# shaderko/velocity-asr

Measured on AMD Instinct MI355X. Metric: audio-sec/sec (RTFx) + frames/s, 5M model batch=32×10s @ 1/2/4/8 MI355X, higher is better.
Workload: dtype f32

## Files before the change

velocity-asr_amd/csrc/gemm_rows.hip:

```cpp
#include <type_traits>

#include "gemm_common.h"
#include "gemm_split.h"

namespace vasr {
namespace {

using namespace gemm;

typedef __attribute__((address_space(3))) void lds_void;

__device__ __forceinline__ void glds16(const void* src, void* dst_base) {
    const unsigned lds = (unsigned)(uintptr_t)(lds_void*)dst_base;
    unsigned keep;
    asm volatile("s_mov_b32 %0, m0\n\ts_mov_b32 m0, %1\n\ts_nop 0\n\tglobal_load_lds_dwordx4 %2, off\n\ts_mov_b32 m0, %0"
                 : "=&s"(keep) : "s"(lds), "v"(src) : "memory");
}

template <int N>
__device__ __forceinline__ void wait_vmcnt() {
    static_assert(N >= 0 && N < 64, "vmcnt range");
    __builtin_amdgcn_s_waitcnt((N & 15) | ((N >> 4) << 14) | (7 << 4) | (15 << 8));
}

#ifndef VASR_ROWS_ABLATE
#define VASR_ROWS_ABLATE 0
#endif
#ifndef VASR_ROWS_WAVES
#define VASR_ROWS_WAVES 8
#endif
#ifndef VASR_ROWS_DEPTH
#define VASR_ROWS_DEPTH 2
#endif
#ifndef VASR_ROWS_STORE_AUX
#define VASR_ROWS_STORE_AUX 2
#endif
constexpr int RW = VASR_ROWS_WAVES;
constexpr int DEPTH = VASR_ROWS_DEPTH;
constexpr int NSLOT = DEPTH + 1;
#ifndef VASR_ROWS_STORE_WAIT
#define VASR_ROWS_STORE_WAIT 1
#endif
#ifndef VASR_ROWS_MAX_GROUP
#define VASR_ROWS_MAX_GROUP 16
#endif
constexpr int MAX_GROUP = VASR_ROWS_MAX_GROUP;

__device__ __forceinline__ void wait_vmcnt_rt(int n) {
    switch (n) {
#define VASR_W(I) case I: wait_vmcnt<I>(); break;
#define VASR_W8(B) VASR_W(B) VASR_W(B + 1) VASR_W(B + 2) VASR_W(B + 3) VASR_W(B + 4) VASR_W(B + 5) VASR_W(B + 6) VASR_W(B + 7)
        VASR_W8(0) VASR_W8(8) VASR_W8(16) VASR_W8(24) VASR_W8(32) VASR_W8(40) VASR_W8(48) VASR_W8(56)
#undef VASR_W8
#undef VASR_W
        default: wait_vmcnt<0>();
    }
}

#ifdef VASR_ROWS_STAMPS
__device__ unsigned long long* g_rows_stamps;
#define VASR_STAMP(v) const unsigned long long v = __builtin_amdgcn_s_memtime()
#else
#define VASR_STAMP(v)
#endif

constexpr int NST = 16;
constexpr int OOB = 0x7FFFFFFC;

template <int EPI>
__device__ __forceinline__ void rows_epilogue(const GemmParams& p, __amdgpu_buffer_rsrc_t cbuf, int m0, int n0,
                                              const floatx16& acc, int r, int h, const float* __restrict__ bias_s,
                                              const float4* __restrict__ qp_s, int cfirst) {
    const int col = n0 + r;
    const bool col_ok = col < p.N;
    const int lc = col - cfirst;
    const float bv = p.bias ? bias_s[lc] : 0.0f;
    float4 qc = make_float4(0.f, 0.f, 0.f, 0.f);
    if (p.qp) qc = qp_s[lc];
    if constexpr (EPI == VASR_EPI_ARGMAX) {
        const int slot = n0 / 32;
#pragma unroll
        for (int i = 0; i < 16; ++i) {
            const int row = m0 + (i & 3) + 8 * (i >> 2) + 4 * h;
            float v = acc[i];
            if (p.bias) v = v + bv;
            if (p.qp) v = fake_quant(v, qc);
            const unsigned u = __float_as_uint(v);
            const unsigned ord = (u & 0x80000000u) ? ~u : (u | 0x80000000u);
            const unsigned long long k0 = col_ok ? ((unsigned long long)ord << 32) | (0xFFFFFFFFu - (unsigned)col) : 0ull;
            const unsigned long long key = gemm::max_u64_over_32_lanes(k0);
            const int off = (r == 31 && row < p.M) ? (row * (int)p.ldc + slot) * 8 : OOB;
            typedef unsigned u32x2 __attribute__((ext_vector_type(2)));
            const u32x2 kv = {(unsigned)key, (unsigned)(key >> 32)};
            if (!(VASR_ROWS_ABLATE & 2)) __builtin_amdgcn_raw_buffer_store_b64(kv, cbuf, off, 0, VASR_ROWS_STORE_AUX);
        }
        return;
    }
    auto body = [&](auto SPc) {
        constexpr int SP = decltype(SPc)::value;
        const bool sp = SP == 1 || (SP == 2 && col >= p.n_out);
#pragma unroll
        for (int i = 0; i < 16; ++i) {
            const int row = m0 + (i & 3) + 8 * (i >> 2) + 4 * h;
            const bool ok = col_ok && row < p.M;
            float v = acc[i];
            if (p.bias) v = v + bv;
            if (p.qp) v = fake_quant(v, qc);
            if constexpr (EPI == VASR_EPI_GELU) {
                v = gelu_fast(v);
            } else if constexpr (EPI == VASR_EPI_SOFTPLUS_FROM) {
                if constexpr (SP == 1) v = softplus20_fast(v);
                else if constexpr (SP == 2) v = sp ? softplus20_fast(v) : v;
            } else if constexpr (EPI == VASR_EPI_RESIDUAL) {
                v = v + p.aux[(int64_t)min(row, p.M - 1) * p.ld_aux + min(col, p.N - 1)];
            } else if constexpr (EPI == VASR_EPI_GELU_PE) {
                v = gelu_fast(v) + p.aux[(int64_t)min(row, p.M - 1) * p.ld_aux + min(col, p.N - 1)];
            }
            if (!(VASR_ROWS_ABLATE & 2))
                __builtin_amdgcn_raw_buffer_store_b32(__float_as_uint(v), cbuf, ok ? (row * (int)p.ldc + col) * 4 : OOB,
                                                      0, VASR_ROWS_STORE_AUX);
        }
    };
    if constexpr (EPI == VASR_EPI_SOFTPLUS_FROM) {
        if (n0 >= p.n_out) body(std::integral_constant<int, 1>());
        else if (n0 + 32 <= p.n_out) body(std::integral_constant<int, 0>());
        else body(std::integral_constant<int, 2>());
    } else {
        body(std::integral_constant<int, 0>());
    }
}

template <int KS, int EPI>
__global__ __launch_bounds__(64 * RW, 1) void gemm_rows_kernel(GemmParams p, int n_groups, int chunks_per_group) {
    constexpr int CHUNK = KS * 3 * 1024;
    constexpr int DW = 4;
    constexpr int NDMA = 3 * KS / DW;
    static_assert((3 * KS) % DW == 0 && RW % DW == 0, "whole DMA pieces per loader wave");
    __shared__ __attribute__((aligned(16))) char wb0[CHUNK];
    __shared__ __attribute__((aligned(16))) char wb1[CHUNK];
    __shared__ __attribute__((aligned(16))) char wb2[CHUNK];
    __shared__ __attribute__((aligned(16))) char wb3[NSLOT > 3 ? CHUNK : 16];
    __shared__ float bias_s[MAX_GROUP * 32];
    __shared__ float4 qp_s[MAX_GROUP * 32];

    const int nblk = (int)gridDim.x;
    const int id = blockIdx.x;
    const int q8 = nblk / 8, r8 = nblk % 8, xg = id % 8;
    const int w = (xg < r8 ? xg * (q8 + 1) : r8 * (q8 + 1) + (xg - r8) * q8) + id / 8;
    const int rb = w / n_groups, ng = w - rb * n_groups;
    const int NT = (p.N + 31) / 32;
    const int c0 = ng * chunks_per_group;
    const int nc = min(chunks_per_group, NT - c0);
    if (nc <= 0) return;

    const int tid = threadIdx.x;
    const int lane = tid & 63;
    const int wave = tid >> 6;
    const int r = lane & 31, h = lane >> 5;
    const int wave_u = __builtin_amdgcn_readfirstlane(wave);
    const int m0 = rb * 32 * RW + wave * 32;
    const int cfirst = c0 * 32;

    const float* __restrict__ arow = p.A + (int64_t)min(m0 + r, p.M - 1) * p.lda;
    float4 xa[KS][2];
#pragma unroll
    for (int ks = 0; ks < KS; ++ks)
#pragma unroll
        for (int u = 0; u < 2; ++u) {
            const int k = 16 * ks + 8 * h + 4 * u;
            const float4 v = *reinterpret_cast<const float4*>(arow + min(k, p.K - 4));
            xa[ks][u] = k < p.K ? v : make_float4(0.f, 0.f, 0.f, 0.f);
        }
    for (int i = tid; i < nc * 32; i += 64 * RW) {
        const int col = min(cfirst + i, p.N - 1);
        if (p.bias) bias_s[i] = p.bias[col];
        if (p.qp) qp_s[i] = p.qp[col];
    }
    bf16x8 a[KS][3];
#pragma unroll
    for (int ks = 0; ks < KS; ++ks) split8(xa[ks][0], xa[ks][1], a[ks][0], a[ks][1], a[ks][2]);

    const char* __restrict__ Wx = reinterpret_cast<const char*>(p.Wx);
    auto slot = [&](int i) -> char* { return i == 0 ? wb0 : i == 1 ? wb1 : i == 2 ? wb2 : wb3; };
    const bool loader = wave_u < DW;
    auto issue = [&](int j) {
        if (!loader) return;
        const char* src = Wx + (int64_t)(c0 + j) * CHUNK + lane * 16;
        char* dst = slot(j % NSLOT);
#pragma unroll
        for (int i = 0; i < NDMA; ++i) {
            const int piece = i * DW + wave_u;
            glds16(src + piece * 1024, dst + piece * 1024);
        }
    };
    for (int j = 0; j < DEPTH && j < nc; ++j) issue(j);

    const int c_bytes = (EPI == VASR_EPI_ARGMAX ? 8 : 4) * ((p.M - 1) * (int)p.ldc + (EPI == VASR_EPI_ARGMAX ? NT : p.N));
    const __amdgpu_buffer_rsrc_t cbuf = __builtin_amdgcn_make_buffer_rsrc(p.C, 0, c_bytes, 0x00020000);
    floatx16 acc[2];
#ifdef VASR_ROWS_STAMPS
    unsigned long long st_wait = 0, st_bar = 0, st_epi = 0, st_dma = 0, st_mfma = 0;
    VASR_STAMP(st_begin);
#endif
    auto step = [&](auto Sc, int j) {
        constexpr int S = decltype(Sc)::value;
        int n_vm = 0;
        if (!loader && !(VASR_ROWS_ABLATE & 2)) n_vm = VASR_ROWS_STORE_WAIT ? NST * max(0, j - max(j - DEPTH + 1, 1)) : 63;
        VASR_STAMP(t0);
        wait_vmcnt_rt(min(n_vm, 63));
        VASR_STAMP(t1);
        if (!(VASR_ROWS_ABLATE & 8)) __builtin_amdgcn_s_barrier();
        VASR_STAMP(t2);
        const char* wb = slot((VASR_ROWS_ABLATE & 4) ? min(j, DEPTH - 1) : j % NSLOT) + lane * 16;
        bf16x8 wf[2][3];
#pragma unroll
        for (int pl = 0; pl < 3; ++pl) wf[0][pl] = *reinterpret_cast<const bf16x8*>(wb + pl * 1024);
        if (j >= 1) rows_epilogue<EPI>(p, cbuf, m0, (c0 + j - 1) * 32, acc[S ^ 1], r, h, bias_s, qp_s, cfirst);
        VASR_STAMP(t3);
        if (j + DEPTH < nc && !(VASR_ROWS_ABLATE & 4)) issue(j + DEPTH);
        VASR_STAMP(t4);
        floatx16 c;
#pragma unroll
        for (int i = 0; i < 16; ++i) c[i] = 0.f;
#pragma unroll
        for (int ks = 0; ks < KS; ++ks) {
            const int cur = ks & 1;
            if (ks + 1 < KS) {
#pragma unroll
                for (int pl = 0; pl < 3; ++pl)
                    wf[cur ^ 1][pl] = *reinterpret_cast<const bf16x8*>(wb + ((ks + 1) * 3 + pl) * 1024);
            }
            __builtin_amdgcn_sched_barrier(0);
            if constexpr (VASR_ROWS_ABLATE & 1) {
                c[0] += (float)a[ks][0][0] * (float)wf[cur][0][0] + (float)a[ks][2][1] * (float)wf[cur][2][1];
                continue;
            }
            c = __builtin_amdgcn_mfma_f32_32x32x16_bf16(a[ks][2], wf[cur][0], c, 0, 0, 0);
            c = __builtin_amdgcn_mfma_f32_32x32x16_bf16(a[ks][0], wf[cur][2], c, 0, 0, 0);
            c = __builtin_amdgcn_mfma_f32_32x32x16_bf16(a[ks][1], wf[cur][1], c, 0, 0, 0);
            c = __builtin_amdgcn_mfma_f32_32x32x16_bf16(a[ks][1], wf[cur][0], c, 0, 0, 0);
            c = __builtin_amdgcn_mfma_f32_32x32x16_bf16(a[ks][0], wf[cur][1], c, 0, 0, 0);
            c = __builtin_amdgcn_mfma_f32_32x32x16_bf16(a[ks][0], wf[cur][0], c, 0, 0, 0);
            __builtin_amdgcn_sched_barrier(0);
        }
        acc[S] = c;
#ifdef VASR_ROWS_STAMPS
        VASR_STAMP(t5);
        st_wait += t1 - t0;
        st_bar += t2 - t1;
        st_epi += t3 - t2;
        st_dma += t4 - t3;
        st_mfma += t5 - t4;
#endif
    };
    for (int j = 0; j < nc; j += 2) {
        step(std::integral_constant<int, 0>(), j);
        if (j + 1 < nc) step(std::integral_constant<int, 1>(), j + 1);
    }
    const int jl = nc - 1;
    rows_epilogue<EPI>(p, cbuf, m0, (c0 + jl) * 32, (jl & 1) ? acc[1] : acc[0], r, h, bias_s, qp_s, cfirst);
#ifdef VASR_ROWS_STAMPS
    __builtin_amdgcn_s_waitcnt(0);
    VASR_STAMP(st_end);
    if (lane == 0 && g_rows_stamps) {
        unsigned long long* o = g_rows_stamps + ((int64_t)blockIdx.x * RW + wave) * 8;
        o[0] = st_wait; o[1] = st_bar; o[2] = st_epi; o[3] = st_dma; o[4] = st_mfma; o[5] = st_end - st_begin;
        o[6] = (unsigned long long)nc; o[7] = loader ? 1 : 0;
    }
#endif
}

#ifndef VASR_ROWS_ROLES
#define VASR_ROWS_ROLES 1
#endif
#ifndef VASR_ROWS_INTERLEAVE
#define VASR_ROWS_INTERLEAVE 1
#endif
#ifndef VASR_ROWS_EPI_FIRST
#define VASR_ROWS_EPI_FIRST 1
#endif
#ifndef VASR_ROWS_DMA_WAVES
#define VASR_ROWS_DMA_WAVES 4
#endif
constexpr int CWV = 4;
constexpr int MWV = 4;
constexpr int DWV = VASR_ROWS_DMA_WAVES;
constexpr int SWV = DWV == MWV ? MWV : MWV - DWV;
static_assert(DWV == 4 || DWV == 2, "VASR_ROWS_DMA_WAVES: 4 or 2");
constexpr int OOB16 = 0x7FFFFFF0;

__device__ __forceinline__ void role_barrier() {
    asm volatile("" ::: "memory");
    __builtin_amdgcn_s_barrier();
    asm volatile("" ::: "memory");
}

template <int CTRL>
__device__ __forceinline__ float dpp_f32(float v) {
    const int i = (int)__float_as_uint(v);
    return __uint_as_float((unsigned)__builtin_amdgcn_update_dpp(i, i, CTRL, 0xF, 0xF, false));
}

template <int EPI, int SP>
__device__ __forceinline__ float rows_value(const GemmParams& p, float v, float bv, const float4& qc, int row, int col) {
    if (p.bias) v = v + bv;
    if (p.qp) v = fake_quant(v, qc);
    if constexpr (EPI == VASR_EPI_GELU) {
        v = gelu_fast(v);
    } else if constexpr (EPI == VASR_EPI_SOFTPLUS_FROM) {
        if constexpr (SP == 1) v = softplus20_fast(v);
        else if constexpr (SP == 2) v = col >= p.n_out ? softplus20_fast(v) : v;
    } else if constexpr (EPI == VASR_EPI_RESIDUAL) {
        v = v + p.aux[(int64_t)min(row, p.M - 1) * p.ld_aux + min(col, p.N - 1)];
    } else if constexpr (EPI == VASR_EPI_GELU_PE) {
        v = gelu_fast(v) + p.aux[(int64_t)min(row, p.M - 1) * p.ld_aux + min(col, p.N - 1)];
    }
    return v;
}

template <int EPI>
__device__ __forceinline__ void roles_epilogue(const GemmParams& p, __amdgpu_buffer_rsrc_t cbuf, int m0, int n0,
                                               const float* __restrict__ tile, int lane, bool wide,
                                               const float* __restrict__ bias_s, const float4* __restrict__ qp_s,
                                               int cfirst) {
    const int rl = lane >> 3, c4 = 4 * (lane & 7);
    const int col0 = n0 + c4;
    const int lc = col0 - cfirst;
    float bv[4] = {0.f, 0.f, 0.f, 0.f};
    if (p.bias) {
        const float4 b = *reinterpret_cast<const float4*>(bias_s + lc);
        bv[0] = b.x; bv[1] = b.y; bv[2] = b.z; bv[3] = b.w;
    }
    float4 qc[4];
#pragma unroll
    for (int e = 0; e < 4; ++e) qc[e] = p.qp ? qp_s[lc + e] : make_float4(0.f, 0.f, 0.f, 0.f);
    if constexpr (EPI == VASR_EPI_ARGMAX) {
        const int slot = n0 / 32;
#pragma unroll
        for (int s = 0; s < 4; ++s) {
            const int row = m0 + 8 * s + rl;
            const float4 x = *reinterpret_cast<const float4*>(tile + (8 * s + rl) * 32 + c4);
            const float xv[4] = {x.x, x.y, x.z, x.w};
            unsigned long long key = 0ull;
#pragma unroll
            for (int e = 0; e < 4; ++e) {
                float v = xv[e];
                if (p.bias) v = v + bv[e];
                if (p.qp) v = fake_quant(v, qc[e]);
                const unsigned u = __float_as_uint(v);
                const unsigned ord = (u & 0x80000000u) ? ~u : (u | 0x80000000u);
                const unsigned long long k =
                    col0 + e < p.N ? ((unsigned long long)ord << 32) | (0xFFFFFFFFu - (unsigned)(col0 + e)) : 0ull;
                key = k > key ? k : key;
            }
            unsigned long long o = gemm::dpp_u64<0xB1, 0xF>(key);
            key = o > key ? o : key;
            o = gemm::dpp_u64<0x4E, 0xF>(key);
            key = o > key ? o : key;
            o = gemm::dpp_u64<0x141, 0xF>(key);
            key = o > key ? o : key;
            const int off = (c4 == 0 && row < p.M) ? (row * (int)p.ldc + slot) * 8 : OOB16;
            typedef unsigned u32x2 __attribute__((ext_vector_type(2)));
            const u32x2 kv = {(unsigned)key, (unsigned)(key >> 32)};
            __builtin_amdgcn_raw_buffer_store_b64(kv, cbuf, off, 0, VASR_ROWS_STORE_AUX);
        }
        return;
    }
    if constexpr (EPI == VASR_EPI_LSE) {
        const int slot = n0 / 32;
#pragma unroll
        for (int s = 0; s < 4; ++s) {
            const int row = m0 + 8 * s + rl;
            const float4 x = *reinterpret_cast<const float4*>(tile + (8 * s + rl) * 32 + c4);
            const float xv[4] = {x.x, x.y, x.z, x.w};
            float v[4];
            float m = -INFINITY;
#pragma unroll
            for (int e = 0; e < 4; ++e) {
                v[e] = col0 + e < p.N ? xv[e] + bv[e] : -INFINITY;
                m = fmaxf(m, v[e]);
            }
            m = fmaxf(m, dpp_f32<0xB1>(m));
            m = fmaxf(m, dpp_f32<0x4E>(m));
            m = fmaxf(m, dpp_f32<0x141>(m));
            const float ms = m == -INFINITY ? 0.f : m;
            float sum = 0.f;
#pragma unroll
            for (int e = 0; e < 4; ++e) sum += fast_exp(v[e] - ms);
            sum += dpp_f32<0xB1>(sum);
            sum += dpp_f32<0x4E>(sum);
            sum += dpp_f32<0x141>(sum);
            const int off = (c4 == 0 && row < p.M) ? (row * (int)p.ldc + slot) * 8 : OOB16;
            typedef unsigned u32x2 __attribute__((ext_vector_type(2)));
            const u32x2 kv = {__float_as_uint(m), __float_as_uint(sum)};
            __builtin_amdgcn_raw_buffer_store_b64(kv, cbuf, off, 0, VASR_ROWS_STORE_AUX);
        }
        return;
    }
    if constexpr (EPI == VASR_EPI_ARGMAX_LSE) {
        const int slot = 2 * (n0 / 32);
#pragma unroll
        for (int s = 0; s < 4; ++s) {
            const int row = m0 + 8 * s + rl;
            const float4 x = *reinterpret_cast<const float4*>(tile + (8 * s + rl) * 32 + c4);
            const float xv[4] = {x.x, x.y, x.z, x.w};
            unsigned long long key = 0ull;
            float v[4];
            float m = -INFINITY;
#pragma unroll
            for (int e = 0; e < 4; ++e) {
                float kvl = xv[e];
                if (p.bias) kvl = kvl + bv[e];
                const unsigned u = __float_as_uint(kvl);
                const unsigned ord = (u & 0x80000000u) ? ~u : (u | 0x80000000u);
                const unsigned long long k =
                    col0 + e < p.N ? ((unsigned long long)ord << 32) | (0xFFFFFFFFu - (unsigned)(col0 + e)) : 0ull;
                key = k > key ? k : key;
                v[e] = col0 + e < p.N ? xv[e] + bv[e] : -INFINITY;
                m = fmaxf(m, v[e]);
            }
            unsigned long long o = gemm::dpp_u64<0xB1, 0xF>(key);
            key = o > key ? o : key;
            o = gemm::dpp_u64<0x4E, 0xF>(key);
            key = o > key ? o : key;
            o = gemm::dpp_u64<0x141, 0xF>(key);
            key = o > key ? o : key;
            m = fmaxf(m, dpp_f32<0xB1>(m));
            m = fmaxf(m, dpp_f32<0x4E>(m));
            m = fmaxf(m, dpp_f32<0x141>(m));
            const float ms = m == -INFINITY ? 0.f : m;
            float sum = 0.f;
#pragma unroll
            for (int e = 0; e < 4; ++e) sum += fast_exp(v[e] - ms);
            sum += dpp_f32<0xB1>(sum);
            sum += dpp_f32<0x4E>(sum);
            sum += dpp_f32<0x141>(sum);
            const bool on = c4 == 0 && row < p.M;
            const int off = on ? (row * (int)p.ldc + slot) * 8 : OOB16;
            typedef unsigned u32x2 __attribute__((ext_vector_type(2)));
            const u32x2 kv = {(unsigned)key, (unsigned)(key >> 32)};
            const u32x2 pv = {__float_as_uint(m), __float_as_uint(sum)};
            __builtin_amdgcn_raw_buffer_store_b64(kv, cbuf, off, 0, VASR_ROWS_STORE_AUX);
            __builtin_amdgcn_raw_buffer_store_b64(pv, cbuf, on ? off + 8 : OOB16, 0, VASR_ROWS_STORE_AUX);
        }
        return;
    }
    auto body = [&](auto SPc, auto Wc) {
        constexpr int SP = decltype(SPc)::value;
        constexpr bool WIDE = decltype(Wc)::value;
#pragma unroll
        for (int s = 0; s < 4; ++s) {
            const int row = m0 + 8 * s + rl;
            const float4 x = *reinterpret_cast<const float4*>(tile + (8 * s + rl) * 32 + c4);
            float v[4] = {x.x, x.y, x.z, x.w};
#pragma unroll
            for (int e = 0; e < 4; ++e) v[e] = rows_value<EPI, SP>(p, v[e], bv[e], qc[e], row, col0 + e);
            if constexpr (WIDE) {
                typedef unsigned u32x4 __attribute__((ext_vector_type(4)));
                const u32x4 d = {__float_as_uint(v[0]), __float_as_uint(v[1]), __float_as_uint(v[2]), __float_as_uint(v[3])};
                const int off = (row < p.M && col0 < p.N) ? (row * (int)p.ldc + col0) * 4 : OOB16;
                if (!(VASR_ROWS_ABLATE & 2) || s == 3) __builtin_amdgcn_raw_buffer_store_b128(d, cbuf, off, 0, VASR_ROWS_STORE_AUX);
            } else {
#pragma unroll
                for (int e = 0; e < 4; ++e)
                    __builtin_amdgcn_raw_buffer_store_b32(__float_as_uint(v[e]), cbuf,
                                                          (row < p.M && col0 + e < p.N) ? (row * (int)p.ldc + col0 + e) * 4 : OOB,
                                                          0, VASR_ROWS_STORE_AUX);
            }
        }
    };
    auto width = [&](auto SPc) {
        if (wide) body(SPc, std::true_type());
        else body(SPc, std::false_type());
    };
    if constexpr (EPI == VASR_EPI_SOFTPLUS_FROM) {
        if (n0 >= p.n_out) width(std::integral_constant<int, 1>());
        else if (n0 + 32 <= p.n_out) width(std::integral_constant<int, 0>());
        else width(std::integral_constant<int, 2>());
    } else {
        width(std::integral_constant<int, 0>());
    }
}

template <int KS, int EPI>
__global__ __launch_bounds__(64 * (CWV + MWV), 1) void gemm_rows_roles_kernel(GemmParams p, int n_groups,
                                                                              int chunks_per_group, int wide) {
    constexpr int CHUNK = KS * 3 * 1024;
    constexpr int NDMA = 3 * KS / DWV;
    static_assert((3 * KS) % DWV == 0, "whole DMA pieces per DMA wave");
    static_assert(DEPTH == 2, "the roles kernel's ring is three slots, two chunks ahead");
    __shared__ __attribute__((aligned(16))) char wb0[CHUNK];
    __shared__ __attribute__((aligned(16))) char wb1[CHUNK];
    __shared__ __attribute__((aligned(16))) char wb2[CHUNK];
    __shared__ __attribute__((aligned(16))) float stage[CWV][2][1024];
    __shared__ __attribute__((aligned(16))) float bias_s[MAX_GROUP * 32];
    __shared__ float4 qp_s[MAX_GROUP * 32];

    const int nblk = (int)gridDim.x;
    const int id = blockIdx.x;
    const int q8 = nblk / 8, r8 = nblk % 8, xg = id % 8;
    const int w = (xg < r8 ? xg * (q8 + 1) : r8 * (q8 + 1) + (xg - r8) * q8) + id / 8;
    const int rb = w / n_groups, ng = w - rb * n_groups;
    const int NT = (p.N + 31) / 32;
    constexpr bool IL = VASR_ROWS_INTERLEAVE != 0;
    const int c0 = IL ? ng : ng * chunks_per_group, cstep = IL ? n_groups : 1;
    const int nc = IL ? (NT - ng + n_groups - 1) / n_groups : min(chunks_per_group, NT - c0);
    if (nc <= 0) return;

    const int tid = threadIdx.x;
    const int lane = tid & 63;
    const int wave_u = __builtin_amdgcn_readfirstlane(tid >> 6);
    auto slot = [&](int i) -> char* { return i == 0 ? wb0 : i == 1 ? wb1 : wb2; };
#ifdef VASR_ROWS_STAMPS
    unsigned long long st_wait = 0, st_bar = 0, st_epi = 0, st_dma = 0, st_mfma = 0;
    VASR_STAMP(st_begin);
#endif

    if (wave_u < CWV) {
        const int r = lane & 31, h = lane >> 5;
        const int m0 = rb * 32 * CWV + wave_u * 32;
        const float* __restrict__ arow = p.A + (int64_t)min(m0 + r, p.M - 1) * p.lda;
        float4 xa[KS][2];
#pragma unroll
        for (int ks = 0; ks < KS; ++ks)
#pragma unroll
            for (int u = 0; u < 2; ++u) {
                const int k = 16 * ks + 8 * h + 4 * u;
                const float4 v = *reinterpret_cast<const float4*>(arow + min(k, p.K - 4));
                xa[ks][u] = k < p.K ? v : make_float4(0.f, 0.f, 0.f, 0.f);
            }
        bf16x8 a[KS][3];
#pragma unroll
        for (int ks = 0; ks < KS; ++ks) split8(xa[ks][0], xa[ks][1], a[ks][0], a[ks][1], a[ks][2]);
        for (int j = 0; j < nc; ++j) {
            VASR_STAMP(t0);
            role_barrier();
            VASR_STAMP(t1);
            const char* wb = slot(j % NSLOT) + lane * 16;
            bf16x8 wf[2][3];
#pragma unroll
            for (int pl = 0; pl < 3; ++pl) wf[0][pl] = *reinterpret_cast<const bf16x8*>(wb + pl * 1024);
            floatx16 c;
#pragma unroll
            for (int i = 0; i < 16; ++i) c[i] = 0.f;
#pragma unroll
            for (int ks = 0; ks < KS; ++ks) {
                const int cur = ks & 1;
                if (ks + 1 < KS) {
#pragma unroll
                    for (int pl = 0; pl < 3; ++pl)
                        wf[cur ^ 1][pl] = *reinterpret_cast<const bf16x8*>(wb + ((ks + 1) * 3 + pl) * 1024);
                }
                __builtin_amdgcn_sched_barrier(0);
                c = __builtin_amdgcn_mfma_f32_32x32x16_bf16(a[ks][2], wf[cur][0], c, 0, 0, 0);
                c = __builtin_amdgcn_mfma_f32_32x32x16_bf16(a[ks][0], wf[cur][2], c, 0, 0, 0);
                c = __builtin_amdgcn_mfma_f32_32x32x16_bf16(a[ks][1], wf[cur][1], c, 0, 0, 0);
                c = __builtin_amdgcn_mfma_f32_32x32x16_bf16(a[ks][1], wf[cur][0], c, 0, 0, 0);
                c = __builtin_amdgcn_mfma_f32_32x32x16_bf16(a[ks][0], wf[cur][1], c, 0, 0, 0);
                c = __builtin_amdgcn_mfma_f32_32x32x16_bf16(a[ks][0], wf[cur][0], c, 0, 0, 0);
                __builtin_amdgcn_sched_barrier(0);
            }
            VASR_STAMP(t2);
            float* tile = &stage[wave_u][j & 1][0];
#pragma unroll
            for (int i = 0; i < 16; ++i) tile[((i & 3) + 8 * (i >> 2) + 4 * h) * 32 + r] = c[i];
            __builtin_amdgcn_s_waitcnt(0xC07F);
#ifdef VASR_ROWS_STAMPS
            VASR_STAMP(t3);
            st_bar += t1 - t0;
            st_mfma += t2 - t1;
            st_epi += t3 - t2;
#endif
        }
        VASR_STAMP(t4);
        role_barrier();
#ifdef VASR_ROWS_STAMPS
        VASR_STAMP(t5);
        st_bar += t5 - t4;
#endif
    } else {
        const int mw = wave_u - CWV;
        const bool dma = mw < DWV;
        const bool stores = mw >= MWV - SWV;
        const int sw = mw - (MWV - SWV);
        for (int i = tid - 64 * CWV; i < nc * 32; i += 64 * MWV) {
            const int col = min((c0 + (i >> 5) * cstep) * 32 + (i & 31), p.N - 1);
            if (p.bias) bias_s[i] = p.bias[col];
            if (p.qp) qp_s[i] = p.qp[col];
        }
        const char* __restrict__ Wx = reinterpret_cast<const char*>(p.Wx);
        auto issue = [&](int j) {
            const char* src = Wx + (int64_t)(c0 + j * cstep) * CHUNK + lane * 16;
            char* dst = slot(j % NSLOT);
#pragma unroll
            for (int i = 0; i < NDMA; ++i) {
                const int piece = i * DWV + mw;
                glds16(src + piece * 1024, dst + piece * 1024);
            }
        };
        __builtin_amdgcn_s_waitcnt(0xC07F);
        if (dma)
            for (int j = 0; j < DEPTH && j < nc; ++j) issue(j);
        constexpr bool SLOTS = EPI == VASR_EPI_ARGMAX || EPI == VASR_EPI_LSE || EPI == VASR_EPI_ARGMAX_LSE;
        constexpr int PER = EPI == VASR_EPI_ARGMAX_LSE ? 2 : 1;
        const int c_bytes = (SLOTS ? 8 : 4) * ((p.M - 1) * (int)p.ldc + (SLOTS ? PER * NT : p.N));
        const __amdgpu_buffer_rsrc_t cbuf = __builtin_amdgcn_make_buffer_rsrc(p.C, 0, c_bytes, 0x00020000);
        auto epilogue = [&](int j) {
            if (!stores) return;
            const int n0 = (c0 + j * cstep) * 32;
            for (int cw = sw; cw < CWV; cw += SWV)
                roles_epilogue<EPI>(p, cbuf, rb * 32 * CWV + cw * 32, n0, &stage[cw][j & 1][0], lane, wide != 0,
                                    bias_s, qp_s, n0 - j * 32);
        };
        for (int j = 0; j < nc; ++j) {
            VASR_STAMP(t0);
            if (dma) {
                if (j + 1 < nc) wait_vmcnt<NDMA*(DEPTH - 1)>();
                else wait_vmcnt<0>();
            }
            VASR_STAMP(t1);
            role_barrier();
            VASR_STAMP(t2);
            if (VASR_ROWS_EPI_FIRST && j >= 1) epilogue(j - 1);
            VASR_STAMP(t2e);
            if (dma && j + DEPTH < nc && !(VASR_ROWS_ABLATE & 4)) issue(j + DEPTH);
            VASR_STAMP(t3);
            if (!VASR_ROWS_EPI_FIRST && j >= 1) epilogue(j - 1);
#ifdef VASR_ROWS_STAMPS
            VASR_STAMP(t4);
            st_wait += t1 - t0;
            st_bar += t2 - t1;
            st_dma += t3 - t2e;
            st_epi += (t2e - t2) + (t4 - t3);
#endif
        }
        VASR_STAMP(t5);
        role_barrier();
        VASR_STAMP(t6);
        epilogue(nc - 1);
#ifdef VASR_ROWS_STAMPS
        VASR_STAMP(t7);
        st_bar += t6 - t5;
        st_epi += t7 - t6;
#endif
    }
#ifdef VASR_ROWS_STAMPS
    __builtin_amdgcn_s_waitcnt(0);
    VASR_STAMP(st_end);
    if (lane == 0 && g_rows_stamps) {
        unsigned long long* o = g_rows_stamps + ((int64_t)blockIdx.x * (CWV + MWV) + wave_u) * 8;
        o[0] = st_wait; o[1] = st_bar; o[2] = st_epi; o[3] = st_dma; o[4] = st_mfma; o[5] = st_end - st_begin;
        o[6] = (unsigned long long)nc;
        o[7] = wave_u < CWV ? 2 : DWV == MWV ? 3 : wave_u - CWV < DWV ? 4 : 5;
    }
#endif
}

inline void pick_groups(int row_blocks, int NT, int* groups_out, int* per_out) {
    int groups = 1, per = min(NT, MAX_GROUP), best = -1;
    for (int g = 1; g <= NT; ++g) {
        const int pg = (NT + g - 1) / g;
        if (pg > MAX_GROUP) continue;
        const int gg = (NT + pg - 1) / pg;
        const int cost = ((row_blocks * gg + kCUs - 1) / kCUs) * (pg + 1);
        if (best < 0 || cost < best) {
            best = cost;
            groups = gg;
            per = pg;
        }
    }
    *groups_out = groups;
    *per_out = per;
}

template <int KS>
int launch_roles(const GemmParams& p, int epi, hipStream_t s) {
    const int NT = (p.N + 31) / 32;
    const int row_blocks = (p.M + 32 * CWV - 1) / (32 * CWV);
    int groups, per;
    pick_groups(row_blocks, NT, &groups, &per);
    const int wide = epi != VASR_EPI_ARGMAX && epi != VASR_EPI_LSE && epi != VASR_EPI_ARGMAX_LSE && p.N % 4 == 0 && p.ldc % 4 == 0 && (reinterpret_cast<uintptr_t>(p.C) & 15) == 0;
    const dim3 grid(row_blocks * groups), block(64 * (CWV + MWV));
#define VASR_R(E) hipLaunchKernelGGL((gemm_rows_roles_kernel<KS, E>), grid, block, 0, s, p, groups, per, wide)
    switch (epi) {
        case VASR_EPI_NONE: VASR_R(VASR_EPI_NONE); break;
        case VASR_EPI_GELU: VASR_R(VASR_EPI_GELU); break;
        case VASR_EPI_SOFTPLUS_FROM: VASR_R(VASR_EPI_SOFTPLUS_FROM); break;
        case VASR_EPI_RESIDUAL: VASR_R(VASR_EPI_RESIDUAL); break;
        case VASR_EPI_GELU_PE: VASR_R(VASR_EPI_GELU_PE); break;
        case VASR_EPI_ARGMAX: VASR_R(VASR_EPI_ARGMAX); break;
        case VASR_EPI_LSE: VASR_R(VASR_EPI_LSE); break;
        case VASR_EPI_ARGMAX_LSE: VASR_R(VASR_EPI_ARGMAX_LSE); break;
        default: set_error("vasr_linear_x3_f32: rows engine: epilogue %d not supported", epi); return VASR_EINVAL;
    }
#undef VASR_R
    return launch_status("vasr_linear_x3_f32");
}

template <int KS>
int launch_rows(const GemmParams& p, int epi, hipStream_t s) {
    const int NT = (p.N + 31) / 32;
    const int row_blocks = (p.M + 32 * RW - 1) / (32 * RW);
    int groups, per;
    pick_groups(row_blocks, NT, &groups, &per);
    const dim3 grid(row_blocks * groups), block(64 * RW);
#define VASR_R(E) hipLaunchKernelGGL((gemm_rows_kernel<KS, E>), grid, block, 0, s, p, groups, per)
    switch (epi) {
        case VASR_EPI_NONE: VASR_R(VASR_EPI_NONE); break;
        case VASR_EPI_GELU: VASR_R(VASR_EPI_GELU); break;
        case VASR_EPI_SOFTPLUS_FROM: VASR_R(VASR_EPI_SOFTPLUS_FROM); break;
        case VASR_EPI_RESIDUAL: VASR_R(VASR_EPI_RESIDUAL); break;
        case VASR_EPI_GELU_PE: VASR_R(VASR_EPI_GELU_PE); break;
        case VASR_EPI_ARGMAX: VASR_R(VASR_EPI_ARGMAX); break;
        default: set_error("vasr_linear_x3_f32: rows engine: epilogue %d not supported", epi); return VASR_EINVAL;
    }
#undef VASR_R
    return launch_status("vasr_linear_x3_f32");
}

}

bool rows_x3_selected(int M, int N, int Kp, int64_t ldc, int batch, int epi) {
    if (batch != 1 || Kp > 192 || M <= 0 || epi == VASR_EPI_PAIR_POWER || epi == VASR_EPI_PAIR_FUSION) return false;
    if ((epi == VASR_EPI_LSE || epi == VASR_EPI_ARGMAX_LSE) && !VASR_ROWS_ROLES) return false;
    if (Kp != 128 && Kp != 192) return false;
    const bool slots = epi == VASR_EPI_ARGMAX || epi == VASR_EPI_LSE || epi == VASR_EPI_ARGMAX_LSE;
    if ((int64_t)M * ldc * (slots ? 8 : 4) >= ((int64_t)1 << 31) - 64) return false;
    const int engine = option(VASR_OPT_GEMM_ENGINE);
    if (engine == 1) return false;
    if (engine == 0 && (Kp != 192 || N < 512 || M < 4096 ||
                        !(epi == VASR_EPI_NONE || epi == VASR_EPI_GELU || epi == VASR_EPI_SOFTPLUS_FROM ||
                          epi == VASR_EPI_LSE)))
        return false;
    return true;
}

int launch_rows_x3(const GemmParams& p, int epi, hipStream_t s) {
    const bool roles = VASR_ROWS_ROLES != 0;
    if (roles) return p.Kp == 128 ? launch_roles<8>(p, epi, s) : launch_roles<12>(p, epi, s);
    return p.Kp == 128 ? launch_rows<8>(p, epi, s) : launch_rows<12>(p, epi, s);
}

}

#ifdef VASR_ROWS_STAMPS
VASR_API int vasr_diag_rows_stamps(void* buf) {
    return hipMemcpyToSymbol(HIP_SYMBOL(vasr::g_rows_stamps), &buf, sizeof(buf)) == hipSuccess ? VASR_OK : VASR_EINVAL;
}
#endif
```

Before: 179,600.

## Stage A tile through LDS, double-buffer accumulators, move softplus epilogue math into compute waves

The A-operand prologue now loads coalesced 64-column passes into a swizzled LDS image and then reads per-lane fragments, instead of strided per-row global loads. A double-accumulator path lets compute waves write the previous chunk's tile interleaved with the current chunk's MFMAs, and the store waves lag by two chunks. For the softplus epilogue without fake-quant, bias and softplus are applied by the compute waves, so the store waves only write raw values. This spreads epilogue arithmetic across MFMA latency but adds register pressure and scheduling constraints.

New measurement: 181,800 (median of 6 runs). 1.01x the previous value.

```diff
diff --git a/velocity-asr_amd/csrc/gemm_rows.hip b/velocity-asr_amd/csrc/gemm_rows.hip
--- a/velocity-asr_amd/csrc/gemm_rows.hip
+++ b/velocity-asr_amd/csrc/gemm_rows.hip
@@ -270,6 +270,18 @@
 #endif
 }
 
+#ifndef VASR_ROWS_A_STAGE
+#define VASR_ROWS_A_STAGE 1
+#endif
+#ifndef VASR_ROWS_ACC2
+#define VASR_ROWS_ACC2 0
+#endif
+#ifndef VASR_ROWS_EPI_MATH
+#define VASR_ROWS_EPI_MATH 1
+#endif
+#ifndef VASR_ROWS_HEAD_ARGMAX
+#define VASR_ROWS_HEAD_ARGMAX 0
+#endif
 #ifndef VASR_ROWS_ROLES
 #define VASR_ROWS_ROLES 1
 #endif
@@ -318,7 +330,7 @@
     return v;
 }
 
-template <int EPI>
+template <int EPI, bool RAW = false>
 __device__ __forceinline__ void roles_epilogue(const GemmParams& p, __amdgpu_buffer_rsrc_t cbuf, int m0, int n0,
                                                const float* __restrict__ tile, int lane, bool wide,
                                                const float* __restrict__ bias_s, const float4* __restrict__ qp_s,
@@ -327,13 +339,13 @@
     const int col0 = n0 + c4;
     const int lc = col0 - cfirst;
     float bv[4] = {0.f, 0.f, 0.f, 0.f};
-    if (p.bias) {
+    if (!RAW && p.bias) {
         const float4 b = *reinterpret_cast<const float4*>(bias_s + lc);
         bv[0] = b.x; bv[1] = b.y; bv[2] = b.z; bv[3] = b.w;
     }
     float4 qc[4];
 #pragma unroll
-    for (int e = 0; e < 4; ++e) qc[e] = p.qp ? qp_s[lc + e] : make_float4(0.f, 0.f, 0.f, 0.f);
+    for (int e = 0; e < 4; ++e) qc[e] = !RAW && p.qp ? qp_s[lc + e] : make_float4(0.f, 0.f, 0.f, 0.f);
     if constexpr (EPI == VASR_EPI_ARGMAX) {
         const int slot = n0 / 32;
 #pragma unroll
@@ -453,8 +465,10 @@
             const int row = m0 + 8 * s + rl;
             const float4 x = *reinterpret_cast<const float4*>(tile + (8 * s + rl) * 32 + c4);
             float v[4] = {x.x, x.y, x.z, x.w};
-#pragma unroll
-            for (int e = 0; e < 4; ++e) v[e] = rows_value<EPI, SP>(p, v[e], bv[e], qc[e], row, col0 + e);
+            if constexpr (!RAW) {
+#pragma unroll
+                for (int e = 0; e < 4; ++e) v[e] = rows_value<EPI, SP>(p, v[e], bv[e], qc[e], row, col0 + e);
+            }
             if constexpr (WIDE) {
                 typedef unsigned u32x4 __attribute__((ext_vector_type(4)));
                 const u32x4 d = {__float_as_uint(v[0]), __float_as_uint(v[1]), __float_as_uint(v[2]), __float_as_uint(v[3])};
@@ -473,7 +487,7 @@
         if (wide) body(SPc, std::true_type());
         else body(SPc, std::false_type());
     };
-    if constexpr (EPI == VASR_EPI_SOFTPLUS_FROM) {
+    if constexpr (EPI == VASR_EPI_SOFTPLUS_FROM && !RAW) {
         if (n0 >= p.n_out) width(std::integral_constant<int, 1>());
         else if (n0 + 32 <= p.n_out) width(std::integral_constant<int, 0>());
         else width(std::integral_constant<int, 2>());
@@ -482,13 +496,17 @@
     }
 }
 
-template <int KS, int EPI>
+template <int KS, int EPI, bool CMATH = false>
 __global__ __launch_bounds__(64 * (CWV + MWV), 1) void gemm_rows_roles_kernel(GemmParams p, int n_groups,
                                                                               int chunks_per_group, int wide) {
     constexpr int CHUNK = KS * 3 * 1024;
     constexpr int NDMA = 3 * KS / DWV;
     static_assert((3 * KS) % DWV == 0, "whole DMA pieces per DMA wave");
     static_assert(DEPTH == 2, "the roles kernel's ring is three slots, two chunks ahead");
+    constexpr bool SLOTS = EPI == VASR_EPI_ARGMAX || EPI == VASR_EPI_LSE || EPI == VASR_EPI_ARGMAX_LSE;
+    static_assert(!CMATH || EPI == VASR_EPI_SOFTPLUS_FROM, "compute-wave arithmetic: the softplus epilogue only");
+    constexpr bool ACC2 = VASR_ROWS_ACC2 == 2 || (VASR_ROWS_ACC2 == 1 && SLOTS) || CMATH;
+    constexpr int LAG = ACC2 ? 2 : 1;
     __shared__ __attribute__((aligned(16))) char wb0[CHUNK];
     __shared__ __attribute__((aligned(16))) char wb1[CHUNK];
     __shared__ __attribute__((aligned(16))) char wb2[CHUNK];
@@ -519,19 +537,181 @@
     if (wave_u < CWV) {
         const int r = lane & 31, h = lane >> 5;
         const int m0 = rb * 32 * CWV + wave_u * 32;
-        const float* __restrict__ arow = p.A + (int64_t)min(m0 + r, p.M - 1) * p.lda;
-        float4 xa[KS][2];
-#pragma unroll
-        for (int ks = 0; ks < KS; ++ks)
-#pragma unroll
-            for (int u = 0; u < 2; ++u) {
-                const int k = 16 * ks + 8 * h + 4 * u;
-                const float4 v = *reinterpret_cast<const float4*>(arow + min(k, p.K - 4));
-                xa[ks][u] = k < p.K ? v : make_float4(0.f, 0.f, 0.f, 0.f);
-            }
         bf16x8 a[KS][3];
-#pragma unroll
-        for (int ks = 0; ks < KS; ++ks) split8(xa[ks][0], xa[ks][1], a[ks][0], a[ks][1], a[ks][2]);
+#if VASR_ROWS_A_STAGE
+        {
+            static_assert(KS % 4 == 0, "whole 64-column passes");
+            constexpr int NP = KS / 4;
+            char* img = reinterpret_cast<char*>(&stage[wave_u][0][0]);
+            const int lq = lane >> 4, lc = lane & 15;
+            float4 g[NP][8];
+#pragma unroll
+            for (int i = 0; i < 8; ++i) {
+                const float* __restrict__ src = p.A + (int64_t)min(m0 + 4 * i + lq, p.M - 1) * p.lda;
+#pragma unroll
+                for (int ps = 0; ps < NP; ++ps) {
+                    const int k = 64 * ps + 4 * lc;
+                    const float4 v = *reinterpret_cast<const float4*>(src + min(k, p.K - 4));
+                    g[ps][i] = k < p.K ? v : make_float4(0.f, 0.f, 0.f, 0.f);
+                }
+            }
+#pragma unroll
+            for (int ps = 0; ps < NP; ++ps) {
+#pragma unroll
+                for (int i = 0; i < 8; ++i) {
+                    const int q = 4 * i + lq;
+                    *reinterpret_cast<float4*>(img + q * 256 + ((lc ^ (q & 15)) << 4)) = g[ps][i];
+                }
+                asm volatile("" ::: "memory");
+                __builtin_amdgcn_s_waitcnt(0xC07F);
+                float4 xa[4][2];
+#pragma unroll
+                for (int kk = 0; kk < 4; ++kk)
+#pragma unroll
+                    for (int u = 0; u < 2; ++u)
+                        xa[kk][u] = *reinterpret_cast<const float4*>(img + r * 256 + (((4 * kk + 2 * h + u) ^ (r & 15)) << 4));
+#pragma unroll
+                for (int kk = 0; kk < 4; ++kk)
+                    split8(xa[kk][0], xa[kk][1], a[4 * ps + kk][0], a[4 * ps + kk][1], a[4 * ps + kk][2]);
+                asm volatile("" ::: "memory");
+            }
+        }
+#else
+        {
+            const float* __restrict__ arow = p.A + (int64_t)min(m0 + r, p.M - 1) * p.lda;
+            float4 xa[KS][2];
+#pragma unroll
+            for (int ks = 0; ks < KS; ++ks)
+#pragma unroll
+                for (int u = 0; u < 2; ++u) {
+                    const int k = 16 * ks + 8 * h + 4 * u;
+                    const float4 v = *reinterpret_cast<const float4*>(arow + min(k, p.K - 4));
+                    xa[ks][u] = k < p.K ? v : make_float4(0.f, 0.f, 0.f, 0.f);
+                }
+#pragma unroll
+            for (int ks = 0; ks < KS; ++ks) split8(xa[ks][0], xa[ks][1], a[ks][0], a[ks][1], a[ks][2]);
+        }
+#endif
+#ifdef VASR_ROWS_STAMPS
+        __builtin_amdgcn_sched_barrier(0);
+        VASR_STAMP(t_pro);
+        st_wait = t_pro - st_begin;
+#endif
+        if constexpr (ACC2) {
+            floatx16 acc[2];
+            auto put = [&](auto SPc, float* tile, const floatx16& c, int i, float bv, int col) {
+                float v = c[i];
+                if constexpr (CMATH) {
+                    v = p.bias ? v + bv : v;
+                    if constexpr (decltype(SPc)::value == 1) v = softplus20_fast(v);
+                    else if constexpr (decltype(SPc)::value == 2) v = col >= p.n_out ? softplus20_fast(v) : v;
+                }
+                tile[((i & 3) + 8 * (i >> 2) + 4 * h) * 32 + r] = v;
+            };
+            auto chunk_tables = [&](int j, float& bv, int& col, int& sp) {
+                bv = 0.f; col = 0; sp = 0;
+                if constexpr (CMATH) {
+                    const int n0 = (c0 + j * cstep) * 32;
+                    col = n0 + r;
+                    if (p.bias) bv = bias_s[j * 32 + r];
+                    sp = n0 >= p.n_out ? 1 : n0 + 32 <= p.n_out ? 0 : 2;
+                }
+            };
+            auto first_el = [](int ks) { return CMATH ? 2 * ks : 4 * ks; };
+            auto step = [&](auto Sc, auto Fc, auto SPc, int j, float bv, int col) {
+                constexpr int S = decltype(Sc)::value;
+                constexpr bool FIRST = decltype(Fc)::value;
+                constexpr int SPF = decltype(SPc)::value;
+                VASR_STAMP(t0);
+                role_barrier();
+                VASR_STAMP(t1);
+                const char* wb = slot(j % NSLOT) + lane * 16;
+                float* prev = &stage[wave_u][S ^ 1][0];
+                bf16x8 wf[2][3];
+#pragma unroll
+                for (int pl = 0; pl < 3; ++pl) wf[0][pl] = *reinterpret_cast<const bf16x8*>(wb + pl * 1024);
+                floatx16 c;
+#pragma unroll
+                for (int i = 0; i < 16; ++i) c[i] = 0.f;
+#pragma unroll
+                for (int ks = 0; ks < KS; ++ks) {
+                    const int cur = ks & 1;
+                    if (ks + 1 < KS) {
+#pragma unroll
+                        for (int pl = 0; pl < 3; ++pl)
+                            wf[cur ^ 1][pl] = *reinterpret_cast<const bf16x8*>(wb + ((ks + 1) * 3 + pl) * 1024);
+                    }
+                    __builtin_amdgcn_sched_barrier(0);
+                    c = __builtin_amdgcn_mfma_f32_32x32x16_bf16(a[ks][2], wf[cur][0], c, 0, 0, 0);
+                    c = __builtin_amdgcn_mfma_f32_32x32x16_bf16(a[ks][0], wf[cur][2], c, 0, 0, 0);
+                    c = __builtin_amdgcn_mfma_f32_32x32x16_bf16(a[ks][1], wf[cur][1], c, 0, 0, 0);
+                    c = __builtin_amdgcn_mfma_f32_32x32x16_bf16(a[ks][1], wf[cur][0], c, 0, 0, 0);
+                    c = __builtin_amdgcn_mfma_f32_32x32x16_bf16(a[ks][0], wf[cur][1], c, 0, 0, 0);
+                    c = __builtin_amdgcn_mfma_f32_32x32x16_bf16(a[ks][0], wf[cur][0], c, 0, 0, 0);
+                    if constexpr (!CMATH) __builtin_amdgcn_sched_barrier(0);
+                    if constexpr (!FIRST) {
+                        static_assert(KS == 8 || KS == 12, "16 elements over the k-steps");
+                        const int i0 = min(first_el(ks), 16), i1 = min(first_el(ks + 1), 16);
+#pragma unroll
+                        for (int i = i0; i < i1; ++i) put(SPc, prev, acc[S ^ 1], i, bv, col);
+                        if constexpr (CMATH) {
+                            constexpr int PER = SPF ? 5 : 1;
+#pragma unroll
+                            for (int m = 0; m < 6; ++m) {
+                                __builtin_amdgcn_sched_group_barrier(0x008, 1, 0);
+                                __builtin_amdgcn_sched_group_barrier(0x002, PER, 0);
+                            }
+                            __builtin_amdgcn_sched_group_barrier(0x200, 2, 0);
+                        }
+                    }
+                    if constexpr (CMATH) __builtin_amdgcn_sched_barrier(0);
+                }
+                acc[S] = c;
+                __builtin_amdgcn_s_waitcnt(0xC07F);
+#ifdef VASR_ROWS_STAMPS
+                VASR_STAMP(t2);
+                st_bar += t1 - t0;
+                st_mfma += t2 - t1;
+#endif
+            };
+            auto next = [&](auto Sc, int j) {
+                float bv; int col; int sp;
+                chunk_tables(j - 1, bv, col, sp);
+                if (sp == 1) step(Sc, std::false_type(), std::integral_constant<int, 1>(), j, bv, col);
+                else if (sp == 0) step(Sc, std::false_type(), std::integral_constant<int, 0>(), j, bv, col);
+                else step(Sc, std::false_type(), std::integral_constant<int, 2>(), j, bv, col);
+            };
+            step(std::integral_constant<int, 0>(), std::true_type(), std::integral_constant<int, 0>(), 0, 0.f, 0);
+            for (int j = 1; j < nc; j += 2) {
+                next(std::integral_constant<int, 1>(), j);
+                if (j + 1 < nc) next(std::integral_constant<int, 0>(), j + 1);
+            }
+            VASR_STAMP(t3);
+            role_barrier();
+            VASR_STAMP(t4);
+            float bv; int col; int sp;
+            chunk_tables(nc - 1, bv, col, sp);
+            auto last = [&](auto SPc) {
+                if ((nc - 1) & 1) {
+#pragma unroll
+                    for (int i = 0; i < 16; ++i) put(SPc, &stage[wave_u][1][0], acc[1], i, bv, col);
+                } else {
+#pragma unroll
+                    for (int i = 0; i < 16; ++i) put(SPc, &stage[wave_u][0][0], acc[0], i, bv, col);
+                }
+            };
+            if (sp == 1) last(std::integral_constant<int, 1>());
+            else if (sp == 0) last(std::integral_constant<int, 0>());
+            else last(std::integral_constant<int, 2>());
+            __builtin_amdgcn_s_waitcnt(0xC07F);
+            VASR_STAMP(t5);
+            role_barrier();
+#ifdef VASR_ROWS_STAMPS
+            VASR_STAMP(t6);
+            st_bar += (t4 - t3) + (t6 - t5);
+            st_epi += t5 - t4;
+#endif
+        } else {
         for (int j = 0; j < nc; ++j) {
             VASR_STAMP(t0);
             role_barrier();
@@ -578,6 +758,7 @@
         VASR_STAMP(t5);
         st_bar += t5 - t4;
 #endif
+        }
     } else {
         const int mw = wave_u - CWV;
         const bool dma = mw < DWV;
@@ -601,15 +782,14 @@
         __builtin_amdgcn_s_waitcnt(0xC07F);
         if (dma)
             for (int j = 0; j < DEPTH && j < nc; ++j) issue(j);
-        constexpr bool SLOTS = EPI == VASR_EPI_ARGMAX || EPI == VASR_EPI_LSE || EPI == VASR_EPI_ARGMAX_LSE;
-        constexpr int PER = EPI == VASR_EPI_ARGMAX_LSE ? 2 : 1;
+        constexpr int PER= EPI == VASR_EPI_ARGMAX_LSE ? 2 : 1;
         const int c_bytes = (SLOTS ? 8 : 4) * ((p.M - 1) * (int)p.ldc + (SLOTS ? PER * NT : p.N));
         const __amdgpu_buffer_rsrc_t cbuf = __builtin_amdgcn_make_buffer_rsrc(p.C, 0, c_bytes, 0x00020000);
         auto epilogue = [&](int j) {
             if (!stores) return;
             const int n0 = (c0 + j * cstep) * 32;
             for (int cw = sw; cw < CWV; cw += SWV)
-                roles_epilogue<EPI>(p, cbuf, rb * 32 * CWV + cw * 32, n0, &stage[cw][j & 1][0], lane, wide != 0,
+                roles_epilogue<EPI, CMATH>(p, cbuf, rb * 32 * CWV + cw * 32, n0, &stage[cw][j & 1][0], lane, wide != 0,
                                     bias_s, qp_s, n0 - j * 32);
         };
         for (int j = 0; j < nc; ++j) {
@@ -621,11 +801,11 @@
             VASR_STAMP(t1);
             role_barrier();
             VASR_STAMP(t2);
-            if (VASR_ROWS_EPI_FIRST && j >= 1) epilogue(j - 1);
+            if (VASR_ROWS_EPI_FIRST && j >= LAG) epilogue(j - LAG);
             VASR_STAMP(t2e);
             if (dma && j + DEPTH < nc && !(VASR_ROWS_ABLATE & 4)) issue(j + DEPTH);
             VASR_STAMP(t3);
-            if (!VASR_ROWS_EPI_FIRST && j >= 1) epilogue(j - 1);
+            if (!VASR_ROWS_EPI_FIRST && j >= LAG) epilogue(j - LAG);
 #ifdef VASR_ROWS_STAMPS
             VASR_STAMP(t4);
             st_wait += t1 - t0;
@@ -637,11 +817,22 @@
         VASR_STAMP(t5);
         role_barrier();
         VASR_STAMP(t6);
+        if constexpr (ACC2) {
+            if (nc >= 2) epilogue(nc - 2);
+            VASR_STAMP(t6a);
+            role_barrier();
+#ifdef VASR_ROWS_STAMPS
+            VASR_STAMP(t6b);
+            st_bar += t6b - t6a;
+            st_epi += t6a - t6;
+#endif
+        }
+        VASR_STAMP(t6c);
         epilogue(nc - 1);
 #ifdef VASR_ROWS_STAMPS
         VASR_STAMP(t7);
         st_bar += t6 - t5;
-        st_epi += t7 - t6;
+        st_epi += ACC2 ? t7 - t6c : t7 - t6;
 #endif
     }
 #ifdef VASR_ROWS_STAMPS
@@ -685,7 +876,12 @@
     switch (epi) {
         case VASR_EPI_NONE: VASR_R(VASR_EPI_NONE); break;
         case VASR_EPI_GELU: VASR_R(VASR_EPI_GELU); break;
-        case VASR_EPI_SOFTPLUS_FROM: VASR_R(VASR_EPI_SOFTPLUS_FROM); break;
+        case VASR_EPI_SOFTPLUS_FROM:
+            if (VASR_ROWS_EPI_MATH == 1 && !p.qp)
+                hipLaunchKernelGGL((gemm_rows_roles_kernel<KS, VASR_EPI_SOFTPLUS_FROM, true>), grid, block, 0, s, p, groups, per, wide);
+            else
+                VASR_R(VASR_EPI_SOFTPLUS_FROM);
+            break;
         case VASR_EPI_RESIDUAL: VASR_R(VASR_EPI_RESIDUAL); break;
         case VASR_EPI_GELU_PE: VASR_R(VASR_EPI_GELU_PE); break;
         case VASR_EPI_ARGMAX: VASR_R(VASR_EPI_ARGMAX); break;
@@ -728,9 +924,10 @@
     if ((int64_t)M * ldc * (slots ? 8 : 4) >= ((int64_t)1 << 31) - 64) return false;
     const int engine = option(VASR_OPT_GEMM_ENGINE);
     if (engine == 1) return false;
+    const bool head = VASR_ROWS_HEAD_ARGMAX && VASR_ROWS_ROLES && (epi == VASR_EPI_ARGMAX || epi == VASR_EPI_ARGMAX_LSE);
     if (engine == 0 && (Kp != 192 || N < 512 || M < 4096 ||
                         !(epi == VASR_EPI_NONE || epi == VASR_EPI_GELU || epi == VASR_EPI_SOFTPLUS_FROM ||
-                          epi == VASR_EPI_LSE)))
+                          epi == VASR_EPI_LSE || head)))
         return false;
     return true;
 }
```
